# privacy-scaling-explorations/zkevm-specs

Hardware: AMD Instinct MI355X
Metric: BN254 constraint-rows/sec (higher is better)
Workload: dtype u256 (BN254 Fr: 4xu64 canonical cells, u32-limb Montgomery); 1 GPU; EVM circuit, 2^18 execution steps per GPU, mixed-opcode synthetic trace (BASELINE configs[2]); RW table 816377 rows, bytecode table 43913 rows; steps_per_gpu=262144, rw_rows=816377, bytecode_rows=43913, witness_copies=3

## Files before the change

zkevm_specs_amd/csrc/zkevm_hip.hip:

```cpp
#include <hip/hip_runtime.h>
#include <hip/hip_ext.h>
#include <stdio.h>
#include <string.h>
#include <stdlib.h>
#include <chrono>
#include <string>
#include <vector>

#include <atomic>
#include <mutex>
#include <dlfcn.h>

#include "../../include/zkevm_hip.h"
#include "kernels.hpp"
#include "dist_tally.hpp"
#include "host_index.hpp"
#include "code_dir_build.hpp"

#define ZK_MAX_DEVICES 64
#define ZK_ECDSA_CHUNK_LANES (1ull << 17)
static std::mutex g_dev_mutex;
static hipStream_t g_own_stream[ZK_MAX_DEVICES] = {nullptr};
static hipStream_t g_batch_stream[ZK_MAX_DEVICES][2] = {{nullptr}};
static hipStream_t g_side_stream[ZK_MAX_DEVICES] = {nullptr};
// ... 74 lines not shown
    for (int d = 0; d < ZK_MAX_DEVICES; d++)
        if (g_own_stream[d]) {
            if (hipSetDevice(d) == hipSuccess) {
                (void)hipStreamDestroy(g_own_stream[d]);
                if (g_zero_row[d]) (void)hipFree(g_zero_row[d]);
                if (g_secp_comb[d]) (void)hipFree(g_secp_comb[d]);
                g_secp_comb[d] = nullptr;
            }
            for (int k = 0; k < 2; k++) {
                if (g_batch_stream[d][k]) (void)hipStreamDestroy(g_batch_stream[d][k]);
                g_batch_stream[d][k] = nullptr;
            }
            if (g_side_stream[d]) (void)hipStreamDestroy(g_side_stream[d]);
            g_side_stream[d] = nullptr;
            for (int k = 0; k < 4; k++) {
                if (g_block_stream[d][k]) (void)hipStreamDestroy(g_block_stream[d][k]);
                g_block_stream[d][k] = nullptr;
            }
            g_own_stream[d] = nullptr;
            g_zero_row[d] = nullptr;
        }
    t_stream = nullptr;
    t_device = -1;
}
extern "C" int zk_set_stream(void* st) {
    ARG_TRY(t_device >= 0, "zk_set_stream: call zk_init first");
    t_stream = st ? (hipStream_t)st : g_own_stream[t_device];
    return 0;
}
struct zk_session;
static int session_rebind_stream(zk_session* s, hipStream_t st);
extern "C" int zk_session_set_stream(zk_session* s, void* st) {
    ARG_TRY(s, "zk_session_set_stream: null session");
    return session_rebind_stream(s, (hipStream_t)st);
}

__global__ void tally_reset_kernel(ZkTally* t, u32* counter = nullptr) {
    t[threadIdx.x].fail_count = 0ull;
    t[threadIdx.x].first_fail = ~0ull;
    if (counter && threadIdx.x == 0) *counter = 0u;
}


__global__ void slots_fill_kernel(u32* slots, u32 n) {
    u32 i = blockIdx.x * blockDim.x + threadIdx.x;
    if (i < n) slots[i] = ZK_EMPTY_SLOT;
}

template <u64 (*HASH)(const ZkTable&, u32)>
__global__ void index_build_kernel(ZkTable t, u32* slots, const ZkRwMeta* unless_dense = nullptr) {
    u32 r = blockIdx.x * blockDim.x + threadIdx.x;
    if (r >= t.n || (unless_dense && unless_dense->dense)) return;
    u32 s = (u32)HASH(t, r) & t.mask;
    while (atomicCAS(&slots[s], ZK_EMPTY_SLOT, r) != ZK_EMPTY_SLOT) s = (s + 1) & t.mask;
}
__global__ void slots_fill_unless_dense_kernel(u32* slots, u32 n, const ZkRwMeta* unless_dense) {
    u32 i = blockIdx.x * blockDim.x + threadIdx.x;
    if (i < n && !unless_dense->dense) slots[i] = ZK_EMPTY_SLOT;
}
__global__ void mpt_index_build_kernel(ZkTable t, u32* slots) {
    u32 r = blockIdx.x * blockDim.x + threadIdx.x;
    if (r >= t.n) return;
    const u64 h = state_mpt_key_hash(t, r);
    u32 s = (u32)h & t.mask;
    const u32 v = state_mpt_slot_value(t, r, h);
    while (atomicCAS(&slots[s], ZK_EMPTY_SLOT, v) != ZK_EMPTY_SLOT) s = (s + 1) & t.mask;
}
__global__ void rw_dense_check_kernel(ZkTable t, ZkRwMeta* meta) {
    const u32 r = blockIdx.x * blockDim.x + threadIdx.x;
    if (r >= t.n) return;
    const u64* p = t.cells + (u64)r * RW_NCELLS * 4;
    const u64* p0 = t.cells;
    const u64 base = p0[0];
    const bool ok = (p0[1] | p0[2] | p0[3]) == 0 && (p[1] | p[2] | p[3]) == 0 && p[0] == base + r && base + r >= base;
    if (r == 0) meta->base = base;
    if (!ok) atomicAnd(&meta->dense, 0u);
}

struct EvmSortArgs {
    const u64* steps;
    u32 n_pairs;
    u32* hist;
    u32* hist_next;
    u32* taken;
    uint16_t* bin16;
    u32* group_start;
    u32* perm;
    ZkTally* tally;
    u32* defer_count;
    u32* early_host;
    u32 early_seq;
};
#define EVM_EARLY_WORD 36u
__device__ __forceinline__ void evm_state_hist_body(u32 vblock, const u64* steps, u32 n_pairs, u32* hist, u32* taken, uint16_t* bin16, ZkTally* tally,
                                                    u32* defer_count) {
    __shared__ u32 local[EVM_N_BINS];
    if (vblock == 0) {
        if (threadIdx.x == 0 && defer_count) *defer_count = 0u;
        if (threadIdx.x == 0) {
            tally->fail_count = 0ull;
            tally->first_fail = ~0ull;
        }
        for (u32 k = threadIdx.x; k < EVM_N_BINS; k += blockDim.x) taken[k] = 0;
    }
    for (u32 k = threadIdx.x; k < EVM_N_BINS; k += blockDim.x) local[k] = 0;
    __syncthreads();
    u32 i = vblock * blockDim.x + threadIdx.x;
    if (i < n_pairs) {
        const u32 bin = evm_state_bin((u32)steps[((u64)i * STEP_NCELLS + S_STATE) * 4]);
        bin16[i] = (uint16_t)bin;
        atomicAdd(&local[bin], 1u);
    }
    __syncthreads();
    for (u32 k = threadIdx.x; k < EVM_N_BINS; k += blockDim.x)
        if (local[k]) atomicAdd(&hist[k], local[k]);
}
__global__ void evm_state_hist_kernel(const u64* steps, u32 n_pairs, u32* hist, u32* taken, uint16_t* bin16, ZkTally* tally, u32* defer_count) {
    evm_state_hist_body(blockIdx.x, steps, n_pairs, hist, taken, bin16, tally, defer_count);
}
__device__ __forceinline__ void evm_state_scatter_body(u32 vblock, const uint16_t* bin16, u32 n_pairs, const u32* hist, u32* hist_next,
                                                       u32* taken, u32* group_start, u32* perm, u32* early_host = nullptr, u32 early_seq = 0u) {
    __shared__ u32 sa[EVM_N_BINS], sb[EVM_N_BINS];
    __shared__ u32 local[EVM_N_BINS];
    __shared__ u32 base[EVM_N_BINS];
    __shared__ u32 gsh[EVM_N_GROUPS + 1];
    const u32 k = threadIdx.x;
    u32 c = 0, c_real = 0;
    if (k < EVM_N_BINS) {
        c_real = hist[k];
        c = k < (u32)EVM_GROUP_WARM * 128u ? ((c_real + 63u) & ~63u) : c_real;
        sa[k] = c;
        local[k] = 0;
        if (vblock == 0) hist_next[k] = 0;
    }
    __syncthreads();
    u32* src = sa;
    u32* dst = sb;
    for (u32 off = 1; off < EVM_N_BINS; off <<= 1) {
        if (k < EVM_N_BINS) dst[k] = src[k] + (k >= off ? src[k - off] : 0u);
        __syncthreads();
        u32* t = src; src = dst; dst = t;
    }
    u32 excl = 0;
    if (k < EVM_N_BINS) {
        excl = src[k] - c;
        if (vblock == 0) {
            if ((k & 127u) == 0) group_start[k >> 7] = gsh[k >> 7] = excl;
            if (k == EVM_N_BINS - 1) group_start[EVM_N_GROUPS] = gsh[EVM_N_GROUPS] = src[k];
            for (u32 j = c_real; j < c; j++) perm[excl + j] = EVM_NO_PAIR;
        }
    }
    const u32 i = vblock * blockDim.x + threadIdx.x;
    u32 bin = 0, rank = 0;
    if (i < n_pairs) {
        bin = bin16[i];
        rank = atomicAdd(&local[bin], 1u);
    }
    __syncthreads();
    if (vblock == 0 && k == 0 && early_host) {
        __hip_atomic_store(&early_host[EVM_EARLY_WORD], gsh[EVM_GROUP_WARM + 1] - gsh[EVM_GROUP_WARM], __ATOMIC_RELAXED, __HIP_MEMORY_SCOPE_SYSTEM);
        __hip_atomic_store(&early_host[EVM_EARLY_WORD + 1], gsh[EVM_GROUP_COLD + 1] - gsh[EVM_GROUP_COLD], __ATOMIC_RELAXED, __HIP_MEMORY_SCOPE_SYSTEM);
        __threadfence_system();
        __hip_atomic_store(&early_host[EVM_EARLY_WORD + 2], early_seq, __ATOMIC_RELEASE, __HIP_MEMORY_SCOPE_SYSTEM);
    }
    if (k < EVM_N_BINS && local[k]) base[k] = excl + atomicAdd(&taken[k], local[k]);
    __syncthreads();
    if (i < n_pairs) perm[base[bin] + rank] = i;
}
__global__ __launch_bounds__(1024) void evm_state_scatter_kernel(const uint16_t* bin16, u32 n_pairs, const u32* hist, u32* hist_next,
                                                                 u32* taken, u32* group_start, u32* perm) {
    evm_state_scatter_body(blockIdx.x, bin16, n_pairs, hist, hist_next, taken, group_start, perm);
}
__global__ __launch_bounds__(256) void evm_open_fill_kernel(uint4* ff, u64 n_ff, uint4* zero, u64 n_zero) {
    const u64 stride = (u64)gridDim.x * blockDim.x;
    const uint4 F = make_uint4(~0u, ~0u, ~0u, ~0u), Z = make_uint4(0u, 0u, 0u, 0u);
    for (u64 i = (u64)blockIdx.x * blockDim.x + threadIdx.x; i < n_ff; i += stride) ff[i] = F;
    for (u64 i = (u64)blockIdx.x * blockDim.x + threadIdx.x; i < n_zero; i += stride) zero[i] = Z;
}
__device__ __forceinline__ void rw_prepare_quad(const ZkTable& t, u64* keys, EvmDyn* dyn, u32 vthread) {
    const u32 r = vthread >> 2, q = vthread & 3u;
    const bool in = r < t.n;
    uint4 c0 = make_uint4(0, 0, 0, 0), c1 = c0, c2 = c0;
    u64 base = 0;
    u32 flags = 3u;
    if (in) {
        const uint4* p = reinterpret_cast<const uint4*>(t.cells + (u64)r * RW_NCELLS * 4) + q;
        c0 = p[0];
        c1 = p[4];
        c2 = p[8];
        if (q == 0) {
            base = t.cells[0];
            if (t.flags) flags = t.flags[r];
        }
    }
    bool fit, dense_ok;
    u64 w0 = 0, w1 = 0, w2 = 0, w3 = 0;
    const bool z0hi = (c0.y | c0.z | c0.w) == 0u, z1hi = (c1.y | c1.z | c1.w) == 0u, z2hi = (c2.y | c2.z | c2.w) == 0u;
    const bool z0 = z0hi && c0.x == 0u, z1 = z1hi && c1.x == 0u, z2 = z2hi && c2.x == 0u;
    if (q == 0) {
        const u64 rwc = (u64)c0.x | ((u64)c0.y << 32);
        dense_ok = (c0.z | c0.w) == 0u && rwc == base + r && base + r >= base;
        fit = z1hi && c1.x <= 255u;
        w0 = (u64)(c1.x & 0xffu) << 8 | ((u64)(flags & 3u) << 56) | (1ull << 63);
        w2 = (u64)c2.x | ((u64)c2.y << 32);
        w3 = (u64)c2.z | ((u64)c2.w << 32);
    } else if (q == 1) {
        dense_ok = z0;
        fit = z1 && z2hi;
        w0 = (u64)c2.x << 24;
    } else if (q == 2) {
        dense_ok = true;
        fit = z0hi && c0.x <= 255u && (c1.z | c1.w) == 0u && z2hi && c2.x <= 255u;
        w0 = (u64)(c0.x & 0xffu) | ((u64)(c2.x & 0xffu) << 16);
        w1 = (u64)c1.x | ((u64)c1.y << 32);
    } else {
        dense_ok = true;
        fit = z0 && z1 && z2;
    }
    const u32 qshift = threadIdx.x & 60u;
    const bool fits = ((__ballot(fit) >> qshift) & 0xfull) == 0xfull;
    const unsigned long long nd = __ballot(in && !dense_ok);
    if (nd != 0ull && (threadIdx.x & 63u) == 0) atomicOr(&dyn->rw_sparse, 1u);
    if (r == 0 && q == 0 && in) dyn->rw_base = base;
#pragma unroll
    for (int m = 1; m <= 2; m <<= 1) {
        w0 |= __shfl_xor(w0, m);
        w1 |= __shfl_xor(w1, m);
        w2 |= __shfl_xor(w2, m);
        w3 |= __shfl_xor(w3, m);
    }
    if (!fits) w0 = w1 = w2 = w3 = 0;
    if (in && q < 2) {
        const u64 a = q == 0 ? w0 : w2, b2 = q == 0 ? w1 : w3;
        reinterpret_cast<uint4*>(keys + (u64)r * 4)[q] = make_uint4((u32)a, (u32)(a >> 32), (u32)b2, (u32)(b2 >> 32));
    }
}
#define EVM_OPEN_TABLES 8
struct EvmOpenTables {
    ZkTable t[EVM_OPEN_TABLES];
    u32 block_start[EVM_OPEN_TABLES + 2];
    const u64* wds;
    u32 n_wds;
    EvmDyn* dyn;
    ZkTally* tally;
    ZkTable rw;
    u64* rw_keys;
    u32 dir_block0, rw_block0;
    DirBuild dir;
    const u64* steps;
    u32 n_steps;
    u32* step_recs;
    u32 rec_block0;
    EvmSortArgs sort;
    u32 hist_block0;
    u32 lat_period;
#ifdef ZK_DIAG_P1
    u32 diag_skip;
#endif
};
__device__ __forceinline__ void evm_open_small_tables(const EvmOpenTables& o, u32 block) {
    int k = 0;
#pragma unroll
    for (int j = 1; j <= EVM_OPEN_TABLES; j++) k += block >= o.block_start[j] ? 1 : 0;
    const u32 r = (block - o.block_start[k]) * blockDim.x + threadIdx.x;
    if (k == EVM_OPEN_TABLES) {
        const bool nz = r < o.n_wds && !fr_is_zero(fr_load(o.wds + ((u64)r * 4 + 3) * 4));
        const unsigned long long b = __ballot(nz);
        if (b && (threadIdx.x & 63u) == 0) atomicAdd(&o.dyn->agg_total_wds, (u32)__popcll(b));
        return;
    }
    const ZkTable& t = o.t[k];
    const bool in = r < t.n;
    if (k == 0) {
        bool caller = false, present = false, invalid = false, bad = false;
        if (in) {
            const Fr tag = zk_table_cell(t, r, 1), lo = zk_table_cell(t, r, 3), hi = zk_table_cell(t, r, 4);
            caller = fr_eq_u64(tag, 4);
            present = caller && !(fr_is_zero(lo) && fr_is_zero(hi));
            const bool inv_row = fr_eq_u64(tag, 10);
            bad = inv_row && t.flags && (t.flags[r] & 1u);
            invalid = inv_row && fr_eq_u64(lo, 1);
        }
        const unsigned long long bc = __ballot(caller), bp = __ballot(present), bi = __ballot(invalid), bb = __ballot(bad);
        if ((threadIdx.x & 63u) == 0) {
            if (bc) atomicAdd(&o.dyn->agg_max_txs, (u32)__popcll(bc));
            if (bp) atomicAdd(&o.dyn->agg_total_txs, (u32)__popcll(bp));
            if (bi) atomicAdd(&o.dyn->agg_invalid_txs, (u32)__popcll(bi));
            if (bb) atomicOr(&o.dyn->agg_bad_invalid_rows, 1u);
        }
    }
    if (!in) return;
    u64 h;
    switch (k) {
    case 0: h = tx_key_hash(t, r); break;
    case 1: h = blk_key_hash(t, r); break;
    case 2: h = bc_key_hash(t, r); break;
    case 3: h = copy_key_hash(t, r); break;
    case 4: h = keccak_key_hash(t, r); break;
    case 5: h = expt_key_hash(t, r); break;
    case 6: h = sig_key_hash(t, r); break;
    default: h = ecc_key_hash(t, r); break;
    }
    u32* slots = const_cast<u32*>(t.slots);
    u32 s = (u32)h & t.mask;
    while (atomicCAS(&slots[s], ZK_EMPTY_SLOT, r) != ZK_EMPTY_SLOT) s = (s + 1) & t.mask;
}
__global__ __launch_bounds__(256) void evm_open_phase1_kernel(EvmOpenTables o) {
    if (blockIdx.x == 0 && threadIdx.x < 2) {
        o.tally[threadIdx.x].fail_count = 0ull;
        o.tally[threadIdx.x].first_fail = ~0ull;
    }
    u32 b = blockIdx.x;
    if (o.lat_period > 1u && b < o.rec_block0) {
        const u32 q = b / o.lat_period;
        b = (b == q * o.lat_period && q < o.rw_block0) ? q : o.rw_block0 + b - (q + 1u < o.rw_block0 ? q + 1u : o.rw_block0);
    }
#ifdef ZK_DIAG_P1
    {
        const u32 range = b < o.dir_block0 ? 1u : b < o.hist_block0 ? 2u : b < o.rw_block0 ? 4u : b < o.rec_block0 ? 8u : 16u;
        if (o.diag_skip & range) return;
    }
#endif
    if (b < o.dir_block0) evm_open_small_tables(o, b);
    else if (b < o.hist_block0) dirb_events_row(o.dir, (b - o.dir_block0) * blockDim.x + threadIdx.x);
    else if (b < o.rw_block0) evm_state_hist_body(b - o.hist_block0, o.sort.steps, o.sort.n_pairs, o.sort.hist, o.sort.taken, o.sort.bin16, o.sort.tally, o.sort.defer_count);
    else if (b < o.rec_block0) rw_prepare_quad(o.rw, o.rw_keys, o.dyn, (b - o.rw_block0) * blockDim.x + threadIdx.x);
    else evm_step_record_quad(o.steps, o.n_steps, o.step_recs, (b - o.rec_block0) * blockDim.x + threadIdx.x);
}
#define EVM_OPEN_RW_GENERIC_BLOCKS 64u
#define EVM_OPEN_P2_BLOCK 1024u
__global__ __launch_bounds__(1024) void evm_open_phase2_kernel(EvmOpenTables o, u32 scatter_blocks, u32 dir_blocks, u32 force_generic) {
    if (blockIdx.x < scatter_blocks) {
        evm_state_scatter_body(blockIdx.x, o.sort.bin16, o.sort.n_pairs, o.sort.hist, o.sort.hist_next, o.sort.taken, o.sort.group_start, o.sort.perm,
                               o.sort.early_host, o.sort.early_seq);
        return;
    }
    const u32 b = blockIdx.x - scatter_blocks;
    if (b < dir_blocks) {
        dirb_finalize_entry(o.dir, b * blockDim.x + threadIdx.x);
        return;
    }
    if (!force_generic && o.dyn->rw_sparse == 0u) return;
    if (force_generic && b == dir_blocks && threadIdx.x == 0) o.dyn->rw_sparse = 1u;
    u32* slots = const_cast<u32*>(o.rw.slots);
    const u32 stride = (gridDim.x - scatter_blocks - dir_blocks) * blockDim.x;
    for (u32 r = (b - dir_blocks) * blockDim.x + threadIdx.x; r < o.rw.n; r += stride) {
        u32 s = (u32)rw_key_hash(o.rw, r) & o.rw.mask;
        bool dup = false;
        for (;;) {
            const u32 q = atomicCAS(&slots[s], ZK_EMPTY_SLOT, r);
            if (q == ZK_EMPTY_SLOT) break;
            if (!dup && q < o.rw.n) {
                bool same = true;
                for (int c = 0; c < RW_NCELLS && same; c++) same = fr_eq(zk_table_cell(o.rw, q, c), zk_table_cell(o.rw, r, c));
                dup = same;
            }
            s = (s + 1) & o.rw.mask;
        }
        if (dup) atomicAdd(&o.dyn->agg_rw_dups, 1u);
    }
}

__global__ void fr_op_kernel(int op, const u64* a, const u64* b, u64* out, u64 n) {
    u64 i = (u64)blockIdx.x * blockDim.x + threadIdx.x;
    if (i >= n) return;
    Fr x = fr_load(a + 4 * i), y = fr_load(b + 4 * i), r;
    switch (op) {
    case 0: r = fr_add(x, y); break;
    case 1: r = fr_sub(x, y); break;
    case 2: r = fr_mul(x, y); break;
    case 3: r = fr_mont(x, y); break;
    case 4: r = fr_neg(x); break;
    case 5: r = fr_inv(x); break;
    case 6: r = fr_div(x, y); break;
    case 16: r = sp_mul_p(x, y); break;
    case 17: r = sp_sqr_p(x); break;
    case 18: r = ecc_fq_mul_hook(x, y); break;
    case 26: r = sp_sqrt_p(x); break;
    case 27: r = sp_inv_p(x); break;
    default: r = fr_zero();
    }
    for (int k = 0; k < 4; k++) out[4 * i + k] = (u64)r.v[2 * k] | ((u64)r.v[2 * k + 1] << 32);
}

__global__ __launch_bounds__(64) void evm_publish_kernel(const u32* d, u32* h, u32 seq) {
    const u32 i = threadIdx.x;
    if (i < 32u) __hip_atomic_store(&h[i], d[i], __ATOMIC_RELAXED, __HIP_MEMORY_SCOPE_SYSTEM);
    __threadfence_system();
    if (i == 0u) __hip_atomic_store(&h[32], seq, __ATOMIC_RELEASE, __HIP_MEMORY_SCOPE_SYSTEM);
}
struct EvmResultBlock {
    EvmDyn dyn;
    u32 n_deferred_twin;
    u32 pad0[(64 - sizeof(EvmDyn)) / 4 - 1];
    ZkTally tally[2];
    u32 group_start[EVM_N_GROUPS + 1];
    u32 pad1[8 - (EVM_N_GROUPS + 1)];
};
static_assert(sizeof(EvmDyn) <= 64 && sizeof(EvmResultBlock) == 128, "EvmResultBlock layout");
enum SessionKind { SESSION_PIA = 18, SESSION_EXA = 17, SESSION_TXA = 16, SESSION_WITHDRAWAL = 15, SESSION_REKEY = 14, SESSION_PICOPY = 13, SESSION_PI = 12, SESSION_CPA = 11, SESSION_STATE = 1, SESSION_EVM = 2, SESSION_BYTECODE = 3, SESSION_EXP = 4, SESSION_COPY = 5, SESSION_SIGN = 6, SESSION_KECCAK = 7, SESSION_ASSIGN = 8, SESSION_ECDSA = 9, SESSION_BCA = 10 };

struct zk_session {
    SessionKind kind;
    int device = t_device;
    hipStream_t stream = t_stream;
    u64 n = 0;
    u64 eval_lo = 0, eval_hi = 0;
    std::vector<void*> owned;
    std::vector<int> owned_class;
    ZkTally* d_tally = nullptr;
    u32* d_status = nullptr;
    bool status_external = false;
    std::vector<hipEvent_t> ev;
    u32 launches = 0;
    u32 tally_pass = 0;
    ZkTally* tally_last = nullptr;
    StateArgs state;
    EvmArgs evm;
    BytecodeArgs bytecode;
    ExpArgs exp;
    CopyArgs copy;
    SignArgs sign;
    KeccakGenArgs keccak_gen;
    AssignArgs assign;
    EcdsaArgs ecdsa;
    BcaArgs bca;
    CpaArgs cpa;
    PiArgs pi;
    PiCopyArgs picopy;
    WithdrawalArgs withdrawal;
    TxAssignArgs txa;
    ExaArgs exa;
    u64 exa_n_table = 0;
    PiaArgs pia;
    PiaSizes pia_sizes;
    KeccakGenArgs pia_kgen;
    u64 pia_host[4] = {0, 0, 0, 0};
    RekeyArgs rekey;
    RwkPlan rekey_plan_host;
    bool assign_from_rw = false;
    bool fused_order_ready = false;
    bool fused_verify = false;
    u32* rekey_status = nullptr;
    u64 cpa_n_table = 0, cpa_n_rw = 0;
    u32* d_hist = nullptr;
    u32* d_cursor = nullptr;
    u32* d_hist2 = nullptr;
    uint16_t* d_bin16 = nullptr;
    u32 evm_pass = 0;
    bool perm_ready = false;
    u32 evm_tally_idx = 0;
    bool perm_valid = false;
    int evm_ranges_known = 0;
    bool evm_warm_empty = false, evm_cold_empty = false;
    u32 evm_warm_lanes = 0;
    bool deferred_pending = false;
    u32* last_status = nullptr;
    u32* d_group_start = nullptr;
    u32* d_perm = nullptr;
    hipEvent_t ev_open0 = nullptr, ev_open1 = nullptr;
    bool side_stream = false;
    hipEvent_t ev_fork = nullptr, ev_join = nullptr;
    void* d_result = nullptr;
    void* h_result = nullptr;
    u32 publish_seq = 0;
    bool publish_enqueued = false;
    u32* h_result_dev = nullptr;
    u32 early_seq = 0;
    bool tail_pending = false;
    u32 tail_cold_grid = 0;
    u32* tail_status = nullptr;
    hipEvent_t tail_e1 = nullptr;
    bool stream_drained = false;
};

static const int MAX_EVENT_PAIRS = 256;

static int session_rebind_stream(zk_session* s, hipStream_t st) {
    HIP_TRY(hipSetDevice(s->device));
    if (!st) st = g_own_stream[s->device];
    if (st == s->stream) return 0;
    HIP_TRY(hipStreamSynchronize(s->stream));
    s->stream = st;
    return 0;
}

#define ZK_ARENA_CLASSES 48
struct DevArena {
    std::mutex m;
    std::vector<void*> free_[ZK_ARENA_CLASSES];
    std::vector<hipEvent_t> events;
    std::vector<void*> pinned;
    size_t cached_bytes = 0;
};
static DevArena g_arena[ZK_MAX_DEVICES];
static size_t arena_limit() {
    static const size_t lim = [] { const char* e = getenv("ZK_ARENA_MAX_BYTES"); return e ? (size_t)strtoull(e, nullptr, 10) : ((size_t)16 << 30); }();
    return lim;
}
static bool arena_off() {
    static const bool off = [] { const char* e = getenv("ZK_NO_ARENA"); return e && e[0] == '1'; }();
    return off;
}
static int arena_class(size_t bytes) {
    int c = 8;
    while (((size_t)1 << c) < bytes) c++;
    return c;
}
static int arena_take(int device, size_t bytes, void** p, int* cls) {
    const int c = arena_class(bytes ? bytes : 16);
    *cls = c;
    if (!arena_off() && c < ZK_ARENA_CLASSES) {
        DevArena& A = g_arena[device];
        std::lock_guard<std::mutex> lock(A.m);
        if (!A.free_[c].empty()) {
            *p = A.free_[c].back();
            A.free_[c].pop_back();
            A.cached_bytes -= (size_t)1 << c;
            return 0;
        }
    }
    HIP_TRY(hipMalloc(p, arena_off() ? (bytes ? bytes : 16) : ((size_t)1 << c)));
    return 0;
}
static void arena_give(int device, void* p, int cls) {
    if (!arena_off() && cls < ZK_ARENA_CLASSES) {
        DevArena& A = g_arena[device];
        std::lock_guard<std::mutex> lock(A.m);
        if (A.cached_bytes + ((size_t)1 << cls) <= arena_limit()) {
            A.free_[cls].push_back(p);
            A.cached_bytes += (size_t)1 << cls;
// ... 118 lines not shown
    hipLaunchKernelGGL(tally_reset_kernel, dim3(1), dim3(2), 0, s->stream, s->d_tally, (u32*)nullptr);
    s->tally_last = s->d_tally;
    rc = dev_alloc(s, (void**)&s->d_status, (size_t)s->n * sizeof(u32));
    if (rc) return rc;
    HIP_TRY(hipMemsetAsync(s->d_status, 0, (size_t)s->n * sizeof(u32), s->stream));
    return 0;
}

extern "C" int zk_close(zk_session* s) {
    if (!s) return 0;
    (void)hipSetDevice(s->device);
    if (!s->stream_drained) (void)hipStreamSynchronize(s->stream);
    for (size_t k = 0; k < s->owned.size(); k++) arena_give(s->device, s->owned[k], s->owned_class[k]);
    {
        DevArena& A = g_arena[s->device];
        std::lock_guard<std::mutex> lock(A.m);
        for (hipEvent_t e : s->ev) A.events.push_back(e);
        if (s->ev_open0) A.events.push_back(s->ev_open0);
        if (s->ev_open1) A.events.push_back(s->ev_open1);
        if (s->ev_fork) A.events.push_back(s->ev_fork);
        if (s->ev_join) A.events.push_back(s->ev_join);
        if (s->h_result) A.pinned.push_back(s->h_result);
    }
    delete s;
    return 0;
}

extern "C" int zk_state_open(const uint64_t* rows, const uint32_t* flags, uint64_t n, const uint64_t* mpt,
                             uint64_t n_mpt, uint32_t opts, zk_session** out) {
    ARG_TRY(t_device >= 0, "zk_state_open: call zk_init first");
    HIP_TRY(hipSetDevice(t_device));
    ARG_TRY(out && rows && n > 0 && n < (1ull << 32), "zk_state_open: bad arguments");
    ARG_TRY(n_mpt < (1ull << 31), "zk_state_open: MPT table too large");
    const bool dev = opts & ZK_OPT_DEVICE_PTRS;
    const bool compact = opts & ZK_OPT_STATE_COMPACT;
    zk_session* s = new zk_session();
    s->kind = SESSION_STATE;
    s->n = n;
    int rc = 0;
    const void* p = nullptr;
    if ((rc = stage(s, rows, (size_t)n * (compact ? 15 : ST_NCELLS) * 32, dev, &p))) goto fail;
    s->state.rows.cells = (const u64*)p;
    s->state.rows.skip = compact ? 42u : 0u;
    if ((rc = stage(s, flags, (size_t)n * 4, dev, &p))) goto fail;
    s->state.rows.flags = (const u32*)p;
    s->state.rows.n = n;
    s->state.eval_lo = 0;
    s->state.eval_hi = n;
    if ((rc = stage(s, mpt, (size_t)n_mpt * MPT_NCELLS * 32, dev, &p))) goto fail;
    s->state.mpt.cells = (const u64*)p;
    s->state.mpt.flags = nullptr;
    s->state.mpt.n = (u32)n_mpt;
    s->state.mpt.ncells = MPT_NCELLS;
    if ((rc = build_index<state_mpt_key_hash>(s, s->state.mpt, true))) goto fail;
    if ((rc = session_common_init(s))) goto fail;
    *out = s;
    return 0;
fail:
    zk_close(s);
    return rc;
}

static int table_stage(zk_session* s, ZkTable& t, const uint64_t* cells, const uint32_t* flags, uint64_t n,
                       u32 ncells, bool dev) {
    const void* p = nullptr;
    int rc;
    if ((rc = stage(s, cells, (size_t)n * ncells * 32, dev, &p))) return rc;
    t.cells = (const u64*)p;
    if ((rc = stage(s, flags, (size_t)n * 4, dev, &p))) return rc;
    t.flags = (n && flags) ? (const u32*)p : nullptr;
    t.n = (u32)n;
    t.ncells = ncells;
    return 0;
}

#ifndef ZK_HIST_BLOCK
#define ZK_HIST_BLOCK 1024
#endif
static int evm_build_perm(zk_session* s) {
    const u32 n = s->evm.n_pairs;
    u32* h_cur = (s->evm_pass & 1u) ? s->d_hist2 : s->d_hist;
    u32* h_next = (s->evm_pass & 1u) ? s->d_hist : s->d_hist2;
    s->evm_pass++;
    hipLaunchKernelGGL(evm_state_hist_kernel, dim3((n + ZK_HIST_BLOCK - 1) / ZK_HIST_BLOCK), dim3(ZK_HIST_BLOCK), 0, s->stream, s->evm.steps, n, h_cur, s->d_cursor, s->d_bin16, s->d_tally, s->evm.defer_count);
    hipLaunchKernelGGL(evm_state_scatter_kernel, dim3((n + 1023) / 1024), dim3(1024), 0, s->stream, s->d_bin16, n, h_cur, h_next, s->d_cursor,
                       s->d_group_start, s->d_perm);
    HIP_TRY(hipGetLastError());
    return 0;
}

static inline u32 index_cap(u64 n) {
    u32 cap = 16;
    while (cap < 2 * n + 2) cap <<= 1;
    return cap;
}

extern "C" int zk_evm_open(const zk_evm_tables* t, uint32_t opts, zk_session** out) {
    ARG_TRY(t_device >= 0, "zk_evm_open: call zk_init first");
    HIP_TRY(hipSetDevice(t_device));
    ARG_TRY(t && out && t->steps && t->n_steps >= 2 && t->n_steps < (1ull << 32), "zk_evm_open: bad arguments");
    ARG_TRY(t->n_rw < (1ull << 31) && t->n_bytecode < (1ull << 31) && t->n_tx < (1ull << 31) && t->n_block < (1ull << 31) &&
            t->n_copy < (1ull << 31) && t->n_keccak < (1ull << 31) && t->n_exp < (1ull << 31) && t->n_withdrawals < (1ull << 31) &&
            t->n_sig < (1ull << 31) && t->n_ecc < (1ull << 31),
            "zk_evm_open: table too large");
    ARG_TRY(t->aux_cells == 0 || (t->aux_cells >= 2 && t->aux_cells <= 64), "zk_evm_open: aux_cells must be 0 (= 2) or 2..64");
    const bool dev = opts & ZK_OPT_DEVICE_PTRS;
    const bool generic = opts & ZK_OPT_GENERIC_INDEX;
    zk_session* s = new zk_session();
    s->kind = SESSION_EVM;
    s->n = t->n_steps - 1;
    s->side_stream = (opts & ZK_OPT_SIDE_STREAM) != 0;
    int rc = 0;
    const void* p = nullptr;
    EvmArgs& E = s->evm;
    if ((rc = stage(s, t->steps, (size_t)t->n_steps * STEP_NCELLS * 32, dev, &p))) goto fail;
    E.steps = (const u64*)p;
    E.n_steps = t->n_steps;
    E.n_pairs = (u32)(t->n_steps - 1);
    if ((rc = table_stage(s, E.rw, t->rw, t->rw_flags, t->n_rw, RW_NCELLS, dev))) goto fail;
    if ((rc = table_stage(s, E.bytecode, t->bytecode, nullptr, t->n_bytecode, BYTECODE_NCELLS, dev))) goto fail;
    if ((rc = table_stage(s, E.tx, t->tx, t->tx_flags, t->n_tx, TX_NCELLS, dev))) goto fail;
    if ((rc = table_stage(s, E.block, t->block, t->block_flags, t->n_block, BLOCK_NCELLS, dev))) goto fail;
    if ((rc = table_stage(s, E.copy, t->copy, nullptr, t->n_copy, COPY_T_NCELLS, dev))) goto fail;
    if ((rc = table_stage(s, E.keccak, t->keccak, nullptr, t->n_keccak, KECCAK_NCELLS, dev))) goto fail;
    if ((rc = table_stage(s, E.exp, t->exp, nullptr, t->n_exp, EXP_T_NCELLS, dev))) goto fail;
    if ((rc = table_stage(s, E.sig, t->sig, nullptr, t->n_sig, SIG_T_NCELLS, dev))) goto fail;
    if ((rc = table_stage(s, E.ecc, t->ecc, nullptr, t->n_ecc, ECC_T_NCELLS, dev))) goto fail;
    if ((rc = table_stage(s, E.withdrawals, t->withdrawals, nullptr, t->n_withdrawals, 4, dev))) goto fail;
    E.withdrawals.slots = nullptr;
    E.withdrawals.mask = 0;
    E.aux = nullptr;
    E.aux_kind = nullptr;
    E.aux_cells = t->aux_cells ? t->aux_cells : 2u;
    if (t->aux && t->aux_kind) {
        if ((rc = stage(s, t->aux, (size_t)t->n_steps * E.aux_cells * 32, dev, &p))) goto fail;
        E.aux = (const u64*)p;
        if ((rc = stage(s, t->aux_kind, (size_t)t->n_steps * 4, dev, &p))) goto fail;
        E.aux_kind = (const u32*)p;
    }
    {
        ZkTable* const small[EVM_OPEN_TABLES] = {&E.tx, &E.block, &E.bytecode, &E.copy, &E.keccak, &E.exp, &E.sig, &E.ecc};
        const bool want_dir = !generic && t->n_bytecode != 0;
        size_t n_ff = 0;
        u32 caps[EVM_OPEN_TABLES];
        for (int k = 0; k < EVM_OPEN_TABLES; k++) { caps[k] = index_cap(small[k]->n); n_ff += caps[k]; }
        const u32 cap_rw = index_cap(E.rw.n), cap_big = want_dir ? index_cap(t->n_bytecode) : 0u;
        n_ff += (size_t)cap_rw + 2 * (size_t)cap_big + (want_dir ? DIRB_SMALL_SLOTS : 0u);
        u32* ff = nullptr;
        if ((rc = dev_alloc(s, (void**)&ff, n_ff * sizeof(u32)))) goto fail;
        u32* cur = ff;
        for (int k = 0; k < EVM_OPEN_TABLES; k++) { small[k]->slots = cur; small[k]->mask = caps[k] - 1; cur += caps[k]; }
        E.rw.slots = cur; E.rw.mask = cap_rw - 1; cur += cap_rw;
        u32* const dir_rep = cur; cur += cap_big;
        u32* const dir_first = cur; cur += cap_big;
        u32* const small_slots = cur;
        const size_t dyn_bytes = 256, hist_bytes = EVM_N_BINS * sizeof(u32), status_bytes = (((size_t)s->n * sizeof(u32)) + 15) & ~(size_t)15;
        const size_t zero_bytes = dyn_bytes + 2 * hist_bytes + status_bytes + 3 * (size_t)cap_big * 4;
        char* zero = nullptr;
        if ((rc = dev_alloc(s, (void**)&zero, zero_bytes))) goto fail;
        EvmResultBlock* const rb = (EvmResultBlock*)zero;
        EvmDyn* dyn = &rb->dyn;
        s->d_result = rb;
        if ((rc = arena_pinned(s->device, &s->h_result))) goto fail;
        {
            void* hd = nullptr;
            if (hipHostGetDevicePointer(&hd, s->h_result, 0) == hipSuccess) s->h_result_dev = (u32*)hd;
            (void)hipGetLastError();
        }
        static_assert(sizeof(EvmResultBlock) <= 256, "the result block outgrew its slot");
        static_assert((EVM_N_BINS * sizeof(u32)) % 16 == 0, "zero region pieces are 16-byte multiples");
        s->d_hist = (u32*)(zero + dyn_bytes);
        s->d_hist2 = (u32*)(zero + dyn_bytes + hist_bytes);
        s->d_status = (u32*)(zero + dyn_bytes + 2 * hist_bytes);
        u32* const dir_last = (u32*)(zero + dyn_bytes + 2 * hist_bytes + status_bytes);
        E.dyn = dyn;
        E.defer_count = &dyn->n_deferred;
        if ((rc = dev_alloc(s, (void**)&E.defer_list, (size_t)E.n_pairs * sizeof(u32)))) goto fail;
        s->d_tally = rb->tally;
        s->tally_last = s->d_tally;
        {
            const u64 n16 = n_ff / 4 + zero_bytes / 16;
            const u32 fill_grid = (u32)(n16 / 256 < 2048 ? (n16 + 255) / 256 : 2048);
            if (arena_event(s->device, &s->ev_open0) || arena_event(s->device, &s->ev_open1)) s->ev_open0 = s->ev_open1 = nullptr;
            hipExtLaunchKernelGGL(evm_open_fill_kernel, dim3(fill_grid ? fill_grid : 1u), dim3(256), 0, s->stream, s->ev_open0, nullptr, 0, (uint4*)ff,
                                  (u64)(n_ff / 4), (uint4*)zero, (u64)(zero_bytes / 16));
        }
        E.rw_dense = 0;
        E.rw_base = 0;
        E.rw_keys = nullptr;
        E.codes.n = 0;
        E.codes.mask = 0;
        E.codes.packed = nullptr;
        E.codes.entries = nullptr;
        E.codes.slots = nullptr;
        E.agg_max_txs = E.agg_total_txs = E.agg_invalid_txs = E.agg_bad_invalid_rows = E.agg_total_wds = E.agg_rw_dups = 0;
        EvmOpenTables o;
        memset(&o, 0, sizeof o);
        u32 blk = 0;
        for (int k = 0; k < EVM_OPEN_TABLES; k++) { o.t[k] = *small[k]; o.block_start[k] = blk; blk += (small[k]->n + 255u) / 256u; }
        o.block_start[EVM_OPEN_TABLES] = blk;
        blk += (u32)((t->n_withdrawals + 255) / 256);
        o.block_start[EVM_OPEN_TABLES + 1] = blk;
        o.wds = E.withdrawals.cells;
        o.n_wds = (u32)t->n_withdrawals;
        o.dyn = dyn;
        o.tally = s->d_tally;
        o.rw = E.rw;
        if (t->n_rw && !generic) {
            u64* d_keys = nullptr;
            if ((rc = dev_alloc(s, (void**)&d_keys, (size_t)t->n_rw * 32))) goto fail;
            E.rw_keys = d_keys;
            o.rw_keys = d_keys;
        }
        const u32 rw_row_blocks = o.rw_keys ? (u32)((t->n_rw + 63) / 64) : 0u;
        o.dir_block0 = blk;
        u32 dir_row_blocks = 0;
        if (want_dir) {
            DirBuild& d = o.dir;
            d.rows = E.bytecode.cells;
            d.n = (u32)t->n_bytecode;
            d.rep = dir_rep;
            d.first = dir_first;
            d.last = dir_last;
            d.runs = dir_last + cap_big;
            d.bad = dir_last + 2 * (size_t)cap_big;
            d.big_mask = cap_big - 1;
            d.small_slots = small_slots;
            d.dyn = dyn;
            if ((rc = dev_alloc(s, (void**)&d.packed, (size_t)d.n * sizeof(uint16_t)))) goto fail;
            if ((rc = dev_alloc(s, (void**)&d.entries, (size_t)DIRB_MAX_ENTRIES * sizeof(ZkCodeEntry)))) goto fail;
            if ((rc = dev_alloc(s, (void**)&d.list, (size_t)DIRB_MAX_ENTRIES * 4))) goto fail;
            dir_row_blocks = (d.n + 255u) / 256u;
            E.codes.entries = d.entries;
            E.codes.slots = d.small_slots;
            E.codes.packed = d.packed;
        }
        if ((rc = dev_alloc(s, (void**)&s->d_cursor, EVM_N_BINS * sizeof(u32)))) goto fail;
        if ((rc = dev_alloc(s, (void**)&s->d_bin16, (size_t)E.n_pairs * sizeof(uint16_t)))) goto fail;
        s->d_group_start = rb->group_start;
        if ((rc = dev_alloc(s, (void**)&s->d_perm, ((size_t)E.n_pairs + EVM_PERM_PAD + 2 * EVM_HOT_BLOCK) * sizeof(u32)))) goto fail;
        const bool sorted = !(opts & ZK_OPT_NO_STATE_SORT);
        o.hist_block0 = o.dir_block0 + dir_row_blocks;
        u32 hist_blocks = 0, scatter_blocks = 0;
        if (sorted) {
            o.sort.steps = E.steps; o.sort.n_pairs = E.n_pairs; o.sort.hist = s->d_hist; o.sort.hist_next = s->d_hist2;
            o.sort.taken = s->d_cursor; o.sort.bin16 = s->d_bin16; o.sort.group_start = s->d_group_start; o.sort.perm = s->d_perm;
            o.sort.tally = s->d_tally;
            o.sort.defer_count = E.defer_count;
            if ((opts & ZK_OPT_SINGLE_PASS) && s->h_result_dev && evm_lazy_tail_enabled() && !(opts & ZK_OPT_SIDE_STREAM)) {
                static std::atomic<u32> g_early_seq{0};
                u32 q = ++g_early_seq;
                if (!q) q = ++g_early_seq;
                __atomic_store_n(&((u32*)s->h_result)[EVM_EARLY_WORD + 2], 0u, __ATOMIC_RELEASE);
                s->early_seq = q;
                o.sort.early_host = s->h_result_dev;
                o.sort.early_seq = q;
            }
            hist_blocks = (E.n_pairs + 255u) / 256u;
            scatter_blocks = (E.n_pairs + EVM_OPEN_P2_BLOCK - 1u) / EVM_OPEN_P2_BLOCK;
            s->evm_pass = 1;
            s->perm_ready = true;
        }
        o.rw_block0 = o.hist_block0 + hist_blocks;
        o.rec_block0 = o.rw_block0 + rw_row_blocks;
        u32 rec_blocks = 0;
        E.step_recs = nullptr;
        if (!(opts & ZK_OPT_SINGLE_PASS)) {
            u32* recs = nullptr;
            if ((rc = dev_alloc(s, (void**)&recs, (size_t)t->n_steps * EVM_REC_WORDS * sizeof(u32)))) goto fail;
            o.steps = E.steps; o.n_steps = (u32)t->n_steps; o.step_recs = recs;
            E.step_recs = recs;
            rec_blocks = (u32)((t->n_steps + 63) / 64);
        }
        const u32 grid1 = o.rec_block0 + rec_blocks;
        {
            static const u32 spread = [] { const char* e = getenv("ZK_P1_LAT_SPREAD"); const int v = e ? atoi(e) : 2; return (u32)(v < 0 ? 0 : v); }();
            o.lat_period = (o.rw_block0 && spread) ? o.rec_block0 / (spread * o.rw_block0) : 0u;
        }
#ifdef ZK_DIAG_P1
        if (const char* e = getenv("ZK_DIAG_P1_SKIP")) o.diag_skip = (u32)atoi(e);
#endif
        {
            const u32 dir_blocks = want_dir ? DIRB_MAX_ENTRIES / EVM_OPEN_P2_BLOCK : 0u;
            const u32 rw_blocks = t->n_rw ? EVM_OPEN_RW_GENERIC_BLOCKS : 0u;
            bool phase2 = scatter_blocks + dir_blocks + rw_blocks != 0;
#ifdef ZK_DIAG_P1
            if (o.diag_skip) phase2 = false;
#endif
            hipExtLaunchKernelGGL(evm_open_phase1_kernel, dim3(grid1 ? grid1 : 1u), dim3(256), 0, s->stream, nullptr, phase2 ? nullptr : s->ev_open1, 0, o);
            if (phase2)
                hipExtLaunchKernelGGL(evm_open_phase2_kernel, dim3(scatter_blocks + dir_blocks + rw_blocks), dim3(EVM_OPEN_P2_BLOCK), 0, s->stream, nullptr,
                                      s->ev_open1, 0, o, scatter_blocks, dir_blocks, generic ? 1u : 0u);
        }
        if (hipGetLastError() != hipSuccess) { rc = -2; g_err = "zk_evm_open: a build kernel failed to launch"; goto fail; }
    }
    E.opts = (t->begin_with_first_step ? 1u : 0u) | (t->end_with_last_step ? 2u : 0u);
    E.prof = nullptr;
    if (getenv("ZK_EVM_PROF")) {
        if ((rc = dev_alloc(s, (void**)&E.prof, 1024 * 4 * 8 * sizeof(unsigned long long)))) goto fail;
        if (hipMemsetAsync(E.prof, 0, 1024 * 4 * 8 * sizeof(unsigned long long), s->stream) != hipSuccess) { rc = -2; goto fail; }
    }
    E.perm = (opts & ZK_OPT_NO_STATE_SORT) ? nullptr : s->d_perm;
    *out = s;
    return 0;
fail:
    zk_close(s);
    return rc;
}

static void session_timing(zk_session* s, double pass_ms, double* open_ms, double* span_ms);
static int evm_enqueue_tail(zk_session* s);
static bool evm_publish_enqueue(zk_session* s);
extern "C" int zk_evm_verify(const zk_evm_tables* t, uint32_t opts, uint32_t* status_out, zk_result* result) {
    ARG_TRY(result, "zk_evm_verify: result is null");
    zk_session* s = nullptr;
    const auto h0 = std::chrono::steady_clock::now();
    int rc = zk_evm_open(t, opts | ZK_OPT_SINGLE_PASS, &s);
    if (rc) return rc;
    const auto h1 = std::chrono::steady_clock::now();
    const bool dev = opts & ZK_OPT_DEVICE_PTRS;
    rc = zk_launch(s, (dev && status_out) ? status_out : nullptr);
    const auto h2 = std::chrono::steady_clock::now();
    if (!rc) rc = zk_collect(s, result);
    const auto h3 = std::chrono::steady_clock::now();
    if (!rc) {
        t_timing[1] = result->kernel_ms;
        session_timing(s, result->kernel_ms, &t_timing[0], &t_timing[2]);
        for (int k = 0; k < 3; k++) t_timing_sum[k] += t_timing[k];
        t_timing_count++;
// ... 2556 lines not shown
```

Before: 1.594 billion rows/s.

## Compute per-element bin offsets in histogram pass, drop scatter-side global atomics

The histogram kernel now keeps each element's in-block rank and the block's global base, which it gets from the atomicAdd return on the global histogram, and writes a per-element offset array. The scatter kernel then only needs the exclusive prefix sum plus the stored offset, so it no longer needs the shared-memory rank atomics or the global 'taken' counters and their reset. The scatter block size becomes a compile-time knob, with loops over bins when the block is smaller than the bin count. The cost is an extra n_pairs u32 array written and read back.

```diff
diff --git a/zkevm_specs_amd/csrc/zkevm_hip.hip b/zkevm_specs_amd/csrc/zkevm_hip.hip
--- a/zkevm_specs_amd/csrc/zkevm_hip.hip
+++ b/zkevm_specs_amd/csrc/zkevm_hip.hip
@@ -180,7 +180,7 @@
     u32 n_pairs;
     u32* hist;
     u32* hist_next;
-    u32* taken;
+    u32* off;
     uint16_t* bin16;
     u32* group_start;
     u32* perm;
@@ -190,7 +190,7 @@
     u32 early_seq;
 };
 #define EVM_EARLY_WORD 36u
-__device__ __forceinline__ void evm_state_hist_body(u32 vblock, const u64* steps, u32 n_pairs, u32* hist, u32* taken, uint16_t* bin16, ZkTally* tally,
+__device__ __forceinline__ void evm_state_hist_body(u32 vblock, const u64* steps, u32 n_pairs, u32* hist, u32* off, uint16_t* bin16, ZkTally* tally,
                                                     u32* defer_count) {
     __shared__ u32 local[EVM_N_BINS];
     if (vblock == 0) {
@@ -199,75 +199,74 @@
             tally->fail_count = 0ull;
             tally->first_fail = ~0ull;
         }
-        for (u32 k = threadIdx.x; k < EVM_N_BINS; k += blockDim.x) taken[k] = 0;
     }
     for (u32 k = threadIdx.x; k < EVM_N_BINS; k += blockDim.x) local[k] = 0;
     __syncthreads();
-    u32 i = vblock * blockDim.x + threadIdx.x;
+    const u32 i = vblock * blockDim.x + threadIdx.x;
+    u32 bin = 0, rank = 0;
     if (i < n_pairs) {
-        const u32 bin = evm_state_bin((u32)steps[((u64)i * STEP_NCELLS + S_STATE) * 4]);
+        bin = evm_state_bin((u32)steps[((u64)i * STEP_NCELLS + S_STATE) * 4]);
         bin16[i] = (uint16_t)bin;
-        atomicAdd(&local[bin], 1u);
+        rank = atomicAdd(&local[bin], 1u);
     }
     __syncthreads();
     for (u32 k = threadIdx.x; k < EVM_N_BINS; k += blockDim.x)
-        if (local[k]) atomicAdd(&hist[k], local[k]);
-}
-__global__ void evm_state_hist_kernel(const u64* steps, u32 n_pairs, u32* hist, u32* taken, uint16_t* bin16, ZkTally* tally, u32* defer_count) {
-    evm_state_hist_body(blockIdx.x, steps, n_pairs, hist, taken, bin16, tally, defer_count);
-}
-__device__ __forceinline__ void evm_state_scatter_body(u32 vblock, const uint16_t* bin16, u32 n_pairs, const u32* hist, u32* hist_next,
-                                                       u32* taken, u32* group_start, u32* perm, u32* early_host = nullptr, u32 early_seq = 0u) {
-    __shared__ u32 sa[EVM_N_BINS], sb[EVM_N_BINS];
-    __shared__ u32 local[EVM_N_BINS];
-    __shared__ u32 base[EVM_N_BINS];
+        if (local[k]) local[k] = atomicAdd(&hist[k], local[k]);
+    __syncthreads();
+    if (i < n_pairs) off[i] = local[bin] + rank;
+}
+__global__ void evm_state_hist_kernel(const u64* steps, u32 n_pairs, u32* hist, u32* off, uint16_t* bin16, ZkTally* tally, u32* defer_count) {
+    evm_state_hist_body(blockIdx.x, steps, n_pairs, hist, off, bin16, tally, defer_count);
+}
+#ifndef ZK_SCATTER_BLOCK
+#define ZK_SCATTER_BLOCK 1024
+#endif
+static_assert(ZK_SCATTER_BLOCK >= 64 && ZK_SCATTER_BLOCK <= 1024 && ZK_SCATTER_BLOCK % 64 == 0, "whole wavefronts, one block");
+__device__ __forceinline__ void evm_state_scatter_body(u32 vblock, const uint16_t* bin16, const u32* off, u32 n_pairs, const u32* hist, u32* hist_next,
+                                                       u32* group_start, u32* perm, u32* early_host = nullptr, u32 early_seq = 0u) {
+    constexpr u32 B = ZK_SCATTER_BLOCK, NB = EVM_N_BINS;
+    __shared__ u32 sa[NB], sb[NB];
     __shared__ u32 gsh[EVM_N_GROUPS + 1];
-    const u32 k = threadIdx.x;
-    u32 c = 0, c_real = 0;
-    if (k < EVM_N_BINS) {
-        c_real = hist[k];
-        c = k < (u32)EVM_GROUP_WARM * 128u ? ((c_real + 63u) & ~63u) : c_real;
-        sa[k] = c;
-        local[k] = 0;
+    const u32 i = vblock * B + threadIdx.x;
+    u32 bin = 0, place = 0;
+    if (i < n_pairs) {
+        bin = bin16[i];
+        place = off[i];
+    }
+    for (u32 k = threadIdx.x; k < NB; k += B) {
+        const u32 c_real = hist[k];
+        sa[k] = k < (u32)EVM_GROUP_WARM * 128u ? ((c_real + 63u) & ~63u) : c_real;
         if (vblock == 0) hist_next[k] = 0;
     }
     __syncthreads();
     u32* src = sa;
     u32* dst = sb;
-    for (u32 off = 1; off < EVM_N_BINS; off <<= 1) {
-        if (k < EVM_N_BINS) dst[k] = src[k] + (k >= off ? src[k - off] : 0u);
+    for (u32 d = 1; d < NB; d <<= 1) {
+        for (u32 k = threadIdx.x; k < NB; k += B) dst[k] = src[k] + (k >= d ? src[k - d] : 0u);
         __syncthreads();
         u32* t = src; src = dst; dst = t;
     }
-    u32 excl = 0;
-    if (k < EVM_N_BINS) {
-        excl = src[k] - c;
+    for (u32 k = threadIdx.x; k < NB; k += B) {
+        const u32 incl = src[k], c = incl - (k ? src[k - 1] : 0u), excl = incl - c;
+        dst[k] = excl;
         if (vblock == 0) {
             if ((k & 127u) == 0) group_start[k >> 7] = gsh[k >> 7] = excl;
-            if (k == EVM_N_BINS - 1) group_start[EVM_N_GROUPS] = gsh[EVM_N_GROUPS] = src[k];
-            for (u32 j = c_real; j < c; j++) perm[excl + j] = EVM_NO_PAIR;
-        }
-    }
-    const u32 i = vblock * blockDim.x + threadIdx.x;
-    u32 bin = 0, rank = 0;
-    if (i < n_pairs) {
-        bin = bin16[i];
-        rank = atomicAdd(&local[bin], 1u);
+            if (k == NB - 1) group_start[EVM_N_GROUPS] = gsh[EVM_N_GROUPS] = incl;
+            for (u32 j = hist[k]; j < c; j++) perm[excl + j] = EVM_NO_PAIR;
+        }
     }
     __syncthreads();
-    if (vblock == 0 && k == 0 && early_host) {
+    if (vblock == 0 && threadIdx.x == 0 && early_host) {
         __hip_atomic_store(&early_host[EVM_EARLY_WORD], gsh[EVM_GROUP_WARM + 1] - gsh[EVM_GROUP_WARM], __ATOMIC_RELAXED, __HIP_MEMORY_SCOPE_SYSTEM);
         __hip_atomic_store(&early_host[EVM_EARLY_WORD + 1], gsh[EVM_GROUP_COLD + 1] - gsh[EVM_GROUP_COLD], __ATOMIC_RELAXED, __HIP_MEMORY_SCOPE_SYSTEM);
         __threadfence_system();
         __hip_atomic_store(&early_host[EVM_EARLY_WORD + 2], early_seq, __ATOMIC_RELEASE, __HIP_MEMORY_SCOPE_SYSTEM);
     }
-    if (k < EVM_N_BINS && local[k]) base[k] = excl + atomicAdd(&taken[k], local[k]);
-    __syncthreads();
-    if (i < n_pairs) perm[base[bin] + rank] = i;
-}
-__global__ __launch_bounds__(1024) void evm_state_scatter_kernel(const uint16_t* bin16, u32 n_pairs, const u32* hist, u32* hist_next,
-                                                                 u32* taken, u32* group_start, u32* perm) {
-    evm_state_scatter_body(blockIdx.x, bin16, n_pairs, hist, hist_next, taken, group_start, perm);
+    if (i < n_pairs) perm[dst[bin] + place] = i;
+}
+__global__ __launch_bounds__(ZK_SCATTER_BLOCK) void evm_state_scatter_kernel(const uint16_t* bin16, const u32* off, u32 n_pairs, const u32* hist, u32* hist_next,
+                                                                 u32* group_start, u32* perm) {
+    evm_state_scatter_body(blockIdx.x, bin16, off, n_pairs, hist, hist_next, group_start, perm);
 }
 __global__ __launch_bounds__(256) void evm_open_fill_kernel(uint4* ff, u64 n_ff, uint4* zero, u64 n_zero) {
     const u64 stride = (u64)gridDim.x * blockDim.x;
@@ -421,15 +420,15 @@
 #endif
     if (b < o.dir_block0) evm_open_small_tables(o, b);
     else if (b < o.hist_block0) dirb_events_row(o.dir, (b - o.dir_block0) * blockDim.x + threadIdx.x);
-    else if (b < o.rw_block0) evm_state_hist_body(b - o.hist_block0, o.sort.steps, o.sort.n_pairs, o.sort.hist, o.sort.taken, o.sort.bin16, o.sort.tally, o.sort.defer_count);
+    else if (b < o.rw_block0) evm_state_hist_body(b - o.hist_block0, o.sort.steps, o.sort.n_pairs, o.sort.hist, o.sort.off, o.sort.bin16, o.sort.tally, o.sort.defer_count);
     else if (b < o.rec_block0) rw_prepare_quad(o.rw, o.rw_keys, o.dyn, (b - o.rw_block0) * blockDim.x + threadIdx.x);
     else evm_step_record_quad(o.steps, o.n_steps, o.step_recs, (b - o.rec_block0) * blockDim.x + threadIdx.x);
 }
 #define EVM_OPEN_RW_GENERIC_BLOCKS 64u
-#define EVM_OPEN_P2_BLOCK 1024u
-__global__ __launch_bounds__(1024) void evm_open_phase2_kernel(EvmOpenTables o, u32 scatter_blocks, u32 dir_blocks, u32 force_generic) {
+#define EVM_OPEN_P2_BLOCK ((u32)ZK_SCATTER_BLOCK)
+__global__ __launch_bounds__(ZK_SCATTER_BLOCK) void evm_open_phase2_kernel(EvmOpenTables o, u32 scatter_blocks, u32 dir_blocks, u32 force_generic) {
     if (blockIdx.x < scatter_blocks) {
-        evm_state_scatter_body(blockIdx.x, o.sort.bin16, o.sort.n_pairs, o.sort.hist, o.sort.hist_next, o.sort.taken, o.sort.group_start, o.sort.perm,
+        evm_state_scatter_body(blockIdx.x, o.sort.bin16, o.sort.off, o.sort.n_pairs, o.sort.hist, o.sort.hist_next, o.sort.group_start, o.sort.perm,
                                o.sort.early_host, o.sort.early_seq);
         return;
     }
@@ -542,9 +541,9 @@
     u32* rekey_status = nullptr;
     u64 cpa_n_table = 0, cpa_n_rw = 0;
     u32* d_hist = nullptr;
-    u32* d_cursor = nullptr;
     u32* d_hist2 = nullptr;
     uint16_t* d_bin16 = nullptr;
+    u32* d_off = nullptr;
     u32 evm_pass = 0;
     bool perm_ready = false;
     u32 evm_tally_idx = 0;
@@ -829,8 +828,8 @@
     u32* h_cur = (s->evm_pass & 1u) ? s->d_hist2 : s->d_hist;
     u32* h_next = (s->evm_pass & 1u) ? s->d_hist : s->d_hist2;
     s->evm_pass++;
-    hipLaunchKernelGGL(evm_state_hist_kernel, dim3((n + ZK_HIST_BLOCK - 1) / ZK_HIST_BLOCK), dim3(ZK_HIST_BLOCK), 0, s->stream, s->evm.steps, n, h_cur, s->d_cursor, s->d_bin16, s->d_tally, s->evm.defer_count);
-    hipLaunchKernelGGL(evm_state_scatter_kernel, dim3((n + 1023) / 1024), dim3(1024), 0, s->stream, s->d_bin16, n, h_cur, h_next, s->d_cursor,
+    hipLaunchKernelGGL(evm_state_hist_kernel, dim3((n + ZK_HIST_BLOCK - 1) / ZK_HIST_BLOCK), dim3(ZK_HIST_BLOCK), 0, s->stream, s->evm.steps, n, h_cur, s->d_off, s->d_bin16, s->d_tally, s->evm.defer_count);
+    hipLaunchKernelGGL(evm_state_scatter_kernel, dim3((n + ZK_SCATTER_BLOCK - 1) / ZK_SCATTER_BLOCK), dim3(ZK_SCATTER_BLOCK), 0, s->stream, s->d_bin16, s->d_off, n, h_cur, h_next,
                        s->d_group_start, s->d_perm);
     HIP_TRY(hipGetLastError());
     return 0;
@@ -982,8 +981,8 @@
             E.codes.slots = d.small_slots;
             E.codes.packed = d.packed;
         }
-        if ((rc = dev_alloc(s, (void**)&s->d_cursor, EVM_N_BINS * sizeof(u32)))) goto fail;
         if ((rc = dev_alloc(s, (void**)&s->d_bin16, (size_t)E.n_pairs * sizeof(uint16_t)))) goto fail;
+        if ((rc = dev_alloc(s, (void**)&s->d_off, (size_t)E.n_pairs * sizeof(u32)))) goto fail;
         s->d_group_start = rb->group_start;
         if ((rc = dev_alloc(s, (void**)&s->d_perm, ((size_t)E.n_pairs + EVM_PERM_PAD + 2 * EVM_HOT_BLOCK) * sizeof(u32)))) goto fail;
         const bool sorted = !(opts & ZK_OPT_NO_STATE_SORT);
@@ -991,7 +990,7 @@
         u32 hist_blocks = 0, scatter_blocks = 0;
         if (sorted) {
             o.sort.steps = E.steps; o.sort.n_pairs = E.n_pairs; o.sort.hist = s->d_hist; o.sort.hist_next = s->d_hist2;
-            o.sort.taken = s->d_cursor; o.sort.bin16 = s->d_bin16; o.sort.group_start = s->d_group_start; o.sort.perm = s->d_perm;
+            o.sort.off = s->d_off; o.sort.bin16 = s->d_bin16; o.sort.group_start = s->d_group_start; o.sort.perm = s->d_perm;
             o.sort.tally = s->d_tally;
             o.sort.defer_count = E.defer_count;
             if ((opts & ZK_OPT_SINGLE_PASS) && s->h_result_dev && evm_lazy_tail_enabled() && !(opts & ZK_OPT_SIDE_STREAM)) {
```

Measured after the change: 1.573 billion rows/s. 0.987x the previous value.
